# liuli33/CMLPL

Measured on AMD Instinct MI355X. Metric: HSI patches/sec per training step, higher is better.
Workload: dtype f32 (convolutions: f32 operands as 3 exact bf16 pieces on the bf16 MFMA, 6 of 9 piece products, f32 accumulate, per-product worst case 2^-21 -- conv1's tap loops of the per-sample kernels as 2 fp16 pieces with power-of-two operand scales, 3 piece products, worst case 2^-20 / mean 2^-23, falling back; 1 GPU; B2: synthetic PaviaU-shaped patches 11x11x103, spectrum 103, 9 classes, 128 labelled + 128 unlabelled rows per GPU (batch 256), dual BaseNet2 fwd/bwd + contrastive/mutual losses + bank + Adam, epoch 1 (memory-bank smoothing active), in-kernel PCG4D noise / Philox dropout; global_batch=256, parallelism=dp1

## Files before the change

### cmlpl_amd/csrc/conv0.hip

```cpp
#include "common.hpp"
#include "kernels.hpp"
#include "gemm_tn.hpp"

namespace cmlpl {

constexpr int C0_KMAX = 128;

template <int KCAP>
__global__ __launch_bounds__(256) void conv0_fwd_kernel(const float* __restrict__ xn, const float* __restrict__ w0t,
                                                        long long w0t_ns, const float* __restrict__ b,
                                                        long long pstride, float* __restrict__ a0, int n, int C,
                                                        int HW) {
  extern __shared__ __attribute__((aligned(16))) float wl[];
  const int tid = threadIdx.x, lane = tid & 63, l31 = lane & 31, hh = lane >> 5;
  const int wave = __builtin_amdgcn_readfirstlane(tid >> 6);
  const int net = blockIdx.y;
  const int Cp = (C + 1) & ~1, KK = Cp >> 1;
  const long long M = (long long)n * HW;
  const long long m = ((long long)blockIdx.x * 4 + wave) * 32 + l31;
  const long long mm = (m < M) ? m : 0;
  const int sample = (int)(mm / HW), pix = (int)(mm - (long long)sample * HW);
  const float* ap = xn + ((long long)net * n + sample) * C * HW + pix;
  float av[KCAP];
#pragma unroll
  for (int q = 0; q < KCAP; ++q) {
    const int c = 2 * q + hh;
    const bool ok = (q < KK) && (c < C);
    const float v = ap[(long long)(ok ? c : 0) * HW];
    av[q] = ok ? v : 0.f;
  }
  const float4* wsrc = (const float4*)(w0t + (long long)net * w0t_ns);
  staged_copy<8, float4>(Cp * 16, tid, [&](int i) { return wsrc[i]; }, [&](int i, float4 v) { ((float4*)wl)[i] = v; });
  __syncthreads();
  f32x16 acc0 = zero16(), acc1 = zero16();
#pragma unroll
  for (int q = 0; q < KCAP; ++q) {
    if (q < KK) {
      const int c = 2 * q + hh;
      acc0 = mfma32(av[q], wl[c * 64 + l31], acc0);
      acc1 = mfma32(av[q], wl[c * 64 + 32 + l31], acc1);
    }
  }
  const float* bias = b + (long long)net * pstride;
  const float bv0 = bias[l31], bv1 = bias[32 + l31];
  const long long mbase = ((long long)blockIdx.x * 4 + wave) * 32;
  float* out = a0 + (long long)net * M * 64;
#pragma unroll
  for (int r = 0; r < 16; ++r) {
    const long long mr = mbase + acc_row(r, lane);
    if (mr < M) {
      out[mr * 64 + l31] = acc0[r] + bv0;
      out[mr * 64 + 32 + l31] = acc1[r] + bv1;
    }
  }
}

hipError_t launch_conv0_fwd(int nets, int n, int C, int HW, const float* xn, const float* w0t, long long w0t_ns,
                            const float* b, long long pstride, float* a0, hipStream_t st) {
  const long long M = (long long)n * HW;
  const int KK = ((C + 1) & ~1) / 2;
  if (KK > C0_KMAX) return hipErrorInvalidValue;
  const size_t lds = (size_t)2 * KK * 64 * 4;
  dim3 grid((unsigned)((M + 127) / 128), nets);
  if (KK <= 32)      hipLaunchKernelGGL((conv0_fwd_kernel<32>), grid, dim3(256), lds, st, xn, w0t, w0t_ns, b, pstride, a0, n, C, HW);
  else if (KK <= 64) hipLaunchKernelGGL((conv0_fwd_kernel<64>), grid, dim3(256), lds, st, xn, w0t, w0t_ns, b, pstride, a0, n, C, HW);
  else               hipLaunchKernelGGL((conv0_fwd_kernel<128>), grid, dim3(256), lds, st, xn, w0t, w0t_ns, b, pstride, a0, n, C, HW);
  return hipGetLastError();
}

constexpr int C0A_SP = 132;
struct Conv0aArgs {
  XSrc xs; const float* w0b3; long long w0b3_ns; const float* b; long long pstride;
  float* a0; float* xn;
  int n, C, HW;
};

template <int KQMAX>
__global__ __launch_bounds__(256, KQMAX <= 4 ? 4 : 2) void conv0a_fwd_kernel(Conv0aArgs a) {
  extern __shared__ __attribute__((aligned(16))) float slab[];
  const int tid = threadIdx.x, lane = tid & 63, l31 = lane & 31, hh = lane >> 5;
  const int wave = __builtin_amdgcn_readfirstlane(tid >> 6);
  const int s = blockIdx.y, net = blockIdx.z, p0 = blockIdx.x * 128;
  const int C = a.C, HW = a.HW, KQ0 = (C + 15) >> 4;
  const int npx = (HW - p0 < 128) ? HW - p0 : 128, np8 = npx >> 3;
  const long long per = (long long)C * HW;
  const float* xrow = xsrc_row(a.xs, net, s, per);
  const float sigma = a.xs.sigma;
  const float* nzrow = (sigma != 0.f) ? xsrc_noise_row(a.xs, net, s, per) : nullptr;
  const uint64_t gs = xsrc_global_sample(a.xs, s), rstep = xsrc_step(a.xs);
  float* xnrow = (a.xn != nullptr) ? a.xn + ((long long)net * a.n + s) * per : nullptr;
  const uint4* wq = (const uint4*)(a.w0b3 + (long long)net * a.w0b3_ns) + lane;
  constexpr int NI = (KQMAX * 16 * 16 + 255) / 256;
  const int items = C * np8;
  const uint32_t mg = (np8 <= 1) ? 0u : (uint32_t)((0x100000000ULL + (uint32_t)np8 - 1) / (uint32_t)np8);
  float4 v0[NI], v1[NI];
  int cc[NI], jj[NI];
#pragma unroll
  for (int q = 0; q < NI; ++q) {
    const int it = tid + 256 * q;
    const int itc = it < items ? it : 0;
    cc[q] = mg == 0u ? itc : (int)__umulhi((uint32_t)itc, mg);
    jj[q] = itc - cc[q] * np8;
    const float* src = xrow + (long long)cc[q] * HW + p0 + 8 * jj[q];
    v0[q] = *(const float4*)src; v1[q] = *(const float4*)(src + 4);
  }
  if (sigma != 0.f) {
#pragma unroll
    for (int q = 0; q < NI; ++q) {
      const long long e = (long long)cc[q] * HW + p0 + 8 * jj[q];
      float4 z0, z1;
      if (nzrow != nullptr) { z0 = *(const float4*)(nzrow + e); z1 = *(const float4*)(nzrow + e + 4); }
      else noise_normal8(a.xs.seed, rstep, STREAM_NOISE_XP + net, gs, (uint32_t)(e >> 3), z0, z1);
      v0[q].x = fmaf(z0.x, sigma, v0[q].x); v0[q].y = fmaf(z0.y, sigma, v0[q].y);
      v0[q].z = fmaf(z0.z, sigma, v0[q].z); v0[q].w = fmaf(z0.w, sigma, v0[q].w);
      v1[q].x = fmaf(z1.x, sigma, v1[q].x); v1[q].y = fmaf(z1.y, sigma, v1[q].y);
      v1[q].z = fmaf(z1.z, sigma, v1[q].z); v1[q].w = fmaf(z1.w, sigma, v1[q].w);
    }
  }
#pragma unroll
  for (int q = 0; q < NI; ++q) {
    if (tid + 256 * q < items) {
      float* d = slab + cc[q] * C0A_SP + 8 * jj[q];
      *(float4*)d = v0[q]; *(float4*)(d + 4) = v1[q];
      if (xnrow != nullptr) {
        float* g = xnrow + (long long)cc[q] * HW + p0 + 8 * jj[q];
        *(float4*)g = v0[q]; *(float4*)(g + 4) = v1[q];
      }
    }
  }
  uint4 bw[2][6];
#pragma unroll
  for (int kq = 0; kq < 2; ++kq)
#pragma unroll
    for (int i = 0; i < 6; ++i) bw[kq][i] = wq[(((kq < KQ0 ? kq : 0) * 3 + (i >> 1)) * 2 + (i & 1)) * 64];
  for (int i = C * C0A_SP + tid; i < KQ0 * 16 * C0A_SP; i += 256) slab[i] = 0.f;
  if (npx < 128)
    for (int i = tid; i < C * (128 - npx); i += 256) { const int c = i / (128 - npx); slab[c * C0A_SP + npx + (i - c * (128 - npx))] = 0.f; }
  __syncthreads();
  if (32 * wave >= npx) return;
  f32x16 z0 = zero16(), z1 = zero16();
  const float* ap = slab + 8 * hh * C0A_SP + 32 * wave + l31;
  float rn[8];
#pragma unroll
  for (int j = 0; j < 8; ++j) rn[j] = ap[j * C0A_SP];
#pragma unroll
  for (int kq = 0; kq < KQMAX; ++kq) {
    if (kq < KQ0) {
      uint4 A1, A2, A3;
      a_split(make_float4(rn[0], rn[1], rn[2], rn[3]), make_float4(rn[4], rn[5], rn[6], rn[7]), A1, A2, A3);
      if (kq + 1 < KQ0) {
#pragma unroll
        for (int j = 0; j < 8; ++j) rn[j] = ap[((kq + 1) * 16 + j) * C0A_SP];
      }
      const uint4 (&b)[6] = bw[kq & 1];
      z0 = mfma_b3(A1, A2, A3, b[0], b[2], b[4], z0);
      z1 = mfma_b3(A1, A2, A3, b[1], b[3], b[5], z1);
      if (kq + 2 < KQ0) {
#pragma unroll
        for (int i = 0; i < 6; ++i) bw[kq & 1][i] = wq[(((kq + 2) * 3 + (i >> 1)) * 2 + (i & 1)) * 64];
      }
    }
  }
  const float* bias = a.b + (long long)net * a.pstride;
  const float bv0 = bias[l31], bv1 = bias[32 + l31];
  float* out = a.a0 + (((long long)net * a.n + s) * HW + p0 + 32 * wave) * 64;
#pragma unroll
  for (int r = 0; r < 16; ++r) {
    const int m = acc_row(r, lane);
    if (32 * wave + m < npx) {
      out[(long long)m * 64 + l31] = z0[r] + bv0;
      out[(long long)m * 64 + 32 + l31] = z1[r] + bv1;
    }
  }
}

bool conv0a_ok(int C, int HW) {
  return switches().conv0a != 0 && C >= 1 && C <= 128 && (HW & 7) == 0 && HW >= 8;
}

hipError_t launch_conv0a_fwd(int nets, int n, int C, int HW, const XSrc& xs, const float* w0b3, long long w0b3_ns,
                             const float* b, long long pstride, float* a0, float* xn, hipStream_t st) {
  if (!conv0a_ok(C, HW)) return hipErrorInvalidValue;
  Conv0aArgs a;
  a.xs = xs; a.w0b3 = w0b3; a.w0b3_ns = w0b3_ns; a.b = b; a.pstride = pstride; a.a0 = a0; a.xn = xn;
  a.n = n; a.C = C; a.HW = HW;
  const int KQ0 = (C + 15) / 16;
  const size_t lds = (size_t)KQ0 * 16 * C0A_SP * 4;
  static DevOnce attr_once;
  hipError_t e = ensure_max_lds(attr_once, conv0a_fwd_kernel<4>, conv0a_fwd_kernel<8>);
  if (e != hipSuccess) return e;
  dim3 grid((HW + 127) / 128, n, nets);
  if (KQ0 <= 4) hipLaunchKernelGGL((conv0a_fwd_kernel<4>), grid, dim3(256), lds, st, a);
  else          hipLaunchKernelGGL((conv0a_fwd_kernel<8>), grid, dim3(256), lds, st, a);
  return hipGetLastError();
}

constexpr int C0_MAXT = 4;
constexpr int C0_PB = 8;

typedef __attribute__((address_space(3))) void c0_lds_void;
typedef __attribute__((address_space(1))) const void c0_gbl_void;
template <bool DMA>
__global__ __launch_bounds__(256) void conv0_wgrad_kernel(const float* __restrict__ xn, const float* __restrict__ da0,
                                                          float* __restrict__ part, int n, int C, int HWfull, int G,
                                                          int PS, const uint32_t* __restrict__ zstat,
                                                          const uint32_t* __restrict__ h2flag, long long h2flag_ns) {
  extern __shared__ __attribute__((aligned(16))) float smem[];
  const int tid = threadIdx.x, lane = tid & 63, l31 = lane & 31, hh = lane >> 5;
  const int wave = __builtin_amdgcn_readfirstlane(tid >> 6);
  const int net = blockIdx.y, g = blockIdx.x;
  const int NT = (C + 31) >> 5, Ct = NT * 32;
  const int HW = HWfull / PS;
  const int HWp = DMA ? HW : ((HW + 2) | 1);
  const int SPG = (n + G - 1) / G;
  const int sbeg = g * SPG, send = (sbeg + SPG < n) ? sbeg + SPG : n;
  const int ct = wave & 1, it0 = wave >> 1;
  f32x16 acc[C0_MAXT];
#pragma unroll
  for (int t = 0; t < C0_MAXT; ++t) acc[t] = zero16();
  float dbacc = 0.f;
  for (int i = (DMA ? C * HW : 0) + tid; i < Ct * HWp + 64; i += 256) smem[i] = 0.f;
  const int pairs = (HW + 1) >> 1;

  const bool zflag = zstat != nullptr && h2flag[(long long)net * h2flag_ns] == 0u;
  for (int su = sbeg * PS; su < send * PS; ++su) {
    const int s = su / PS, p0 = (su - s * PS) * HW;
    if (zflag && zstat[(2 * 2 + net) * n + s] == 0u && (zstat[(0 * 2 + net) * n + s] >> 23) < 255u) continue;
    const float* brow = da0 + (((long long)net * n + s) * HWfull + p0) * 64 + ct * 32 + l31;
    float bq[4][C0_PB];
    auto fetch = [&](float (&buf)[C0_PB], int t0) {
#pragma unroll
      for (int q = 0; q < C0_PB; ++q) {
        const int p = 2 * (t0 + q) + hh;
        buf[q] = brow[(long long)(p < HW ? p : 0) * 64];
      }
    };
    fetch(bq[0], 0); fetch(bq[1], C0_PB); fetch(bq[2], 2 * C0_PB);
    __syncthreads();
    const float* xs = xn + ((long long)net * n + s) * C * HWfull + p0;
    if (DMA) {
      const int nf4 = (C * HW) >> 2;
      for (int q = wave; q * 64 < nf4; q += 4) {
        const int f = q * 64 + lane;
        if (f < nf4)
          __builtin_amdgcn_global_load_lds((c0_gbl_void*)(xs + 4 * f), (c0_lds_void*)(smem + q * 256), 16, 0, 0);
      }
      const int rem = C * HW - 4 * nf4;
      if (tid < rem) smem[4 * nf4 + tid] = xs[4 * nf4 + tid];
    } else {
      if ((HW & 3) == 0) {
        const int H4 = HW >> 2;
        staged_copy<8, float4>(C * H4, tid,
                               [&](int i) { const int c = i / H4, q = i - c * H4; return *(const float4*)(xs + (long long)c * HWfull + 4 * q); },
                               [&](int i, float4 v) {
                                 const int c = i / H4, p = 4 * (i - c * H4);
                                 float* d = smem + c * HWp + p;
                                 d[0] = v.x; d[1] = v.y; d[2] = v.z; d[3] = v.w;
                               });
      } else {
        staged_copy<16, float>(C * HW, tid, [&](int i) { const int c = i / HW; return xs[(long long)c * HWfull + (i - c * HW)]; },
                               [&](int i, float v) { const int c = i / HW, p = i - c * HW; smem[c * HWp + p] = v; });
      }
    }
    __syncthreads();
    for (int t1 = 0; t1 < pairs; t1 += 4 * C0_PB) {
#pragma unroll
      for (int u = 0; u < 4; ++u) {
        const int t0 = t1 + u * C0_PB;
        if (t0 + 3 * C0_PB < pairs) fetch(bq[(u + 3) & 3], t0 + 3 * C0_PB);
        if (t0 < pairs) {
          float bv[C0_PB];
#pragma unroll
          for (int q = 0; q < C0_PB; ++q) {
            const int p = 2 * (t0 + q) + hh;
            bv[q] = (t0 + q < pairs && p < HW) ? bq[u][q] : 0.f;
            dbacc += bv[q];
          }
#pragma unroll
          for (int k = 0; k < C0_MAXT; ++k) {
            const int tile = it0 + 2 * k;
            if (tile < NT) {
              const float* xr = smem + (tile * 32 + l31) * HWp + 2 * t0 + hh;
              float av[C0_PB];
#pragma unroll
              for (int q = 0; q < C0_PB; ++q) av[q] = xr[2 * q];
              __builtin_amdgcn_sched_barrier(0);
#pragma unroll
              for (int q = 0; q < C0_PB; ++q) acc[k] = mfma32(av[q], bv[q], acc[k]);
            }
          }
        }
      }
    }
  }
  const int Cw = conv0_partial_rows(C);
  float* pp = part + ((long long)net * G + g) * ((long long)Cw * 64 + 64);
#pragma unroll
  for (int k = 0; k < C0_MAXT; ++k) {
    const int tile = it0 + 2 * k;
    if (tile < NT) {
#pragma unroll
      for (int r = 0; r < 16; ++r) {
        const int row = tile * 32 + acc_row(r, lane);
        if (row < Cw) pp[row * 64 + ct * 32 + l31] = acc[k][r];
      }
    }
  }
  if (it0 == 0) {
    const float tot = dbacc + __shfl_xor(dbacc, 32, 64);
    if (hh == 0) pp[(long long)Cw * 64 + ct * 32 + l31] = tot;
  }
}

__device__ __forceinline__ float4 part_row(const float* p, int g, int G, int PS) {
  uint32_t keep = g < G ? 0xffffffffu : 0u;
  asm volatile("" : "+v"(keep));
  const float4 x = *(const float4*)(p + (size_t)(g < G ? g : 0) * PS);
  return make_float4(__uint_as_float(__float_as_uint(x.x) & keep), __uint_as_float(__float_as_uint(x.y) & keep),
                     __uint_as_float(__float_as_uint(x.z) & keep), __uint_as_float(__float_as_uint(x.w) & keep));
}
__device__ __forceinline__ void add_quad(float4& s, const float4& a, const float4& b, const float4& c, const float4& d) {
  s.x += (a.x + b.x) + (c.x + d.x); s.y += (a.y + b.y) + (c.y + d.y);
  s.z += (a.z + b.z) + (c.z + d.z); s.w += (a.w + b.w) + (c.w + d.w);
}

__device__ __forceinline__ float conv0_fold(const ReduceProb& pr, int eb, int net, float4* red4) {
  const int tid = threadIdx.x, col = tid & 31, h = (tid >> 5) & 1, sl = tid >> 6;
  const int G = pr.G, PS = pr.PS;
  const int e0 = eb + col * 4;
  const float* p = pr.part + (long long)net * G * PS + (e0 < PS ? e0 : 0);
  float4 s = make_float4(0.f, 0.f, 0.f, 0.f);
  for (int g0 = sl + 16 * h; g0 - 16 * h < G; g0 += 128) {
    const float4 a0 = part_row(p, g0, G, PS), a1 = part_row(p, g0 + 4, G, PS);
    const float4 a2 = part_row(p, g0 + 8, G, PS), a3 = part_row(p, g0 + 12, G, PS);
    const float4 b0 = part_row(p, g0 + 32, G, PS), b1 = part_row(p, g0 + 36, G, PS);
    const float4 b2 = part_row(p, g0 + 40, G, PS), b3 = part_row(p, g0 + 44, G, PS);
    const float4 c0 = part_row(p, g0 + 64, G, PS), c1 = part_row(p, g0 + 68, G, PS);
    const float4 c2 = part_row(p, g0 + 72, G, PS), c3 = part_row(p, g0 + 76, G, PS);
    const float4 d0 = part_row(p, g0 + 96, G, PS), d1 = part_row(p, g0 + 100, G, PS);
    const float4 d2 = part_row(p, g0 + 104, G, PS), d3 = part_row(p, g0 + 108, G, PS);
    add_quad(s, a0, a1, a2, a3);
    add_quad(s, b0, b1, b2, b3);
    add_quad(s, c0, c1, c2, c3);
    add_quad(s, d0, d1, d2, d3);
  }
  red4[tid] = s;
  __syncthreads();
  const float* sm = (const float*)red4;
  const int w = tid & 127;
  return ((sm[w] + sm[128 + w]) + (sm[256 + w] + sm[384 + w])) + ((sm[512 + w] + sm[640 + w]) + (sm[768 + w] + sm[896 + w]));
}

__device__ __forceinline__ void partial_reduce_block(const ReduceTable& t, int bx, int net, float (*red)[64]) {
  int pi = 0;
  if (t.count > 1 && bx >= t.p[1].blk0) pi = 1;
  if (t.count > 2 && bx >= t.p[2].blk0) pi = 2;
  const ReduceProb pr = t.p[pi];
  const int tid = threadIdx.x, el = tid & 63, sl = tid >> 6;
  if (t.dyn_cursor != nullptr && bx == 0 && net == 0 && tid == 0) {
    const int c = *t.dyn_cursor + 1;
    *t.dyn_cursor = c;
    const uint4* src = (const uint4*)(t.dyn_table + c);
    uint4* dst = (uint4*)t.dyn_table;
    const uint4 r0 = src[0], r1 = src[1], r2 = src[2], r3 = src[3];
    dst[0] = r0; dst[1] = r1; dst[2] = r2; dst[3] = r3;
  }
  const int G = pr.G, PS = pr.PS;
  const int body = PS - 64;
  if (pr.mode == 0) {
    const int eb = (bx - pr.blk0) * REDUCE_CONV0_EL, e = eb + tid;
    const float sum = conv0_fold(pr, eb, net, (float4*)&red[0][0]);
    if (tid < REDUCE_CONV0_EL && e < PS) {
      if (e >= body) pr.db[(long long)net * t.grad_ns + (e - body)] = sum;
      else if ((e >> 6) < pr.C) pr.dW[(long long)net * t.grad_ns + (e & 63) * pr.C + (e >> 6)] = sum;
    }
    return;
  }
  const int e0 = ((bx - pr.blk0) * 64 + el) * 4;
  const bool ev = e0 < PS;
  const float* p = pr.part + (long long)net * G * PS + (ev ? e0 : 0);
  float4 s0 = make_float4(0.f, 0.f, 0.f, 0.f), s1 = s0;
  for (int g0 = sl; g0 < G; g0 += 64) {
    const float4 a0 = part_row(p, g0, G, PS), a1 = part_row(p, g0 + 4, G, PS);
    const float4 a2 = part_row(p, g0 + 8, G, PS), a3 = part_row(p, g0 + 12, G, PS);
    const float4 a4 = part_row(p, g0 + 16, G, PS), a5 = part_row(p, g0 + 20, G, PS);
    const float4 a6 = part_row(p, g0 + 24, G, PS), a7 = part_row(p, g0 + 28, G, PS);
    const float4 b0 = part_row(p, g0 + 32, G, PS), b1 = part_row(p, g0 + 36, G, PS);
    const float4 b2 = part_row(p, g0 + 40, G, PS), b3 = part_row(p, g0 + 44, G, PS);
    const float4 b4 = part_row(p, g0 + 48, G, PS), b5 = part_row(p, g0 + 52, G, PS);
    const float4 b6 = part_row(p, g0 + 56, G, PS), b7 = part_row(p, g0 + 60, G, PS);
    add_quad(s0, a0, a1, a2, a3); add_quad(s1, a4, a5, a6, a7);
    add_quad(s0, b0, b1, b2, b3); add_quad(s1, b4, b5, b6, b7);
  }
  float4* red4 = (float4*)&red[0][0];
  red4[sl * 64 + el] = make_float4(s0.x + s1.x, s0.y + s1.y, s0.z + s1.z, s0.w + s1.w);
  __syncthreads();
  if (sl == 0 && ev) {
    const float4 a = red4[el], b = red4[64 + el], c = red4[128 + el], d = red4[192 + el];
    const float sum[4] = {(a.x + b.x) + (c.x + d.x), (a.y + b.y) + (c.y + d.y), (a.z + b.z) + (c.z + d.z),
                          (a.w + b.w) + (c.w + d.w)};
#pragma unroll
    for (int j = 0; j < 4; ++j) {
      const int e = e0 + j;
      if (e >= body) {
        pr.db[(long long)net * t.grad_ns + (e - body)] = sum[j];
      } else {
        const int s = e >> 12, ci = (e >> 6) & 63, co = e & 63;
        pr.dW[(long long)net * t.grad_ns + co * 576 + ci * 9 + s] = sum[j];
      }
    }
  }
}

__global__ __launch_bounds__(256) void partial_reduce_kernel(ReduceTable t) {
  __shared__ __attribute__((aligned(16))) float red[16][64];
  partial_reduce_block(t, (int)blockIdx.x, (int)blockIdx.y, red);
}

__global__ __launch_bounds__(256) void reduce_gemm_kernel(ReduceTable t, int reduce_blocks, GemmTN2 g) {
  __shared__ GemmTNShared sh;
  const int bid = (int)blockIdx.x;
  if (bid < reduce_blocks) partial_reduce_block(t, bid % t.total_blocks, bid / t.total_blocks, (float (*)[64])&sh.red[0][0][0]);
  else gemm_tn_block(g, bid - reduce_blocks, sh);
}

__device__ __forceinline__ int red_swz(int col) { return col ^ (((col >> 4) & 7) << 1); }

__device__ __forceinline__ void reduce_adam_block_conv0(const ReduceTable& t, const ReduceProb& pr, int bx, int net,
                                                        float* sm, const AdamFuse& f) {
  const int tid = threadIdx.x;
  const int PS = pr.PS, body = PS - 64;
  const int eb = (bx - pr.blk0) * REDUCE_CONV0_EL, e = eb + tid, c = e >> 6, co = e & 63;
  long long po = -1;
  if (tid < REDUCE_CONV0_EL && e < PS) {
    if (e >= body) po = (pr.db - f.gbase) + (e - body);
    else if (c < pr.C) po = (pr.dW - f.gbase) + (long long)co * pr.C + c;
  }
  float* const pp = f.params + (long long)net * f.pstride;
  float* const pm = f.m + (long long)net * f.pstride;
  float* const pv = f.v + (long long)net * f.pstride;
  const long long o = po < 0 ? 0 : po;
  float mq = pm[o], vq = pv[o];
  const float pq = pp[o];
  const float sum = conv0_fold(pr, eb, net, (float4*)sm);
  if (po < 0) return;
  const_cast<float*>(f.gbase)[(long long)net * t.grad_ns + po] = sum;
  const float pn = adam_update<true, false>(mq, vq, pq, sum, f, 1.f, f.keep);
  pm[po] = mq; pv[po] = vq; pp[po] = pn;
  if (e < body) {
    float* const pkn = f.packed + (long long)net * f.pi.stride;
    pkn[pack_off_w0t() + c * 64 + co] = pn;
    uint32_t pcs[3];
    b3_split(pn, pcs);
    uint16_t* wb = (uint16_t*)(pkn + pack_off_w0b3(f.pi.C, f.pi.bands));
#pragma unroll
    for (int pc = 0; pc < 3; ++pc) wb[conv_b3_index(0, c, co, pc)] = (uint16_t)pcs[pc];
  }
}

__device__ __forceinline__ void reduce_adam_block(const ReduceTable& t, int bx, int net, float* sm, const AdamFuse& f) {
  int pi = 0;
  if (t.count > 1 && bx >= t.p[1].blk0) pi = 1;
  if (t.count > 2 && bx >= t.p[2].blk0) pi = 2;
  const ReduceProb pr = t.p[pi];
  if (pr.mode == 0) { reduce_adam_block_conv0(t, pr, bx, net, sm, f); return; }
  const int tid = threadIdx.x, lane = tid & 63, el = lane, sl = tid >> 6;
  const int G = pr.G, PS = pr.PS, body = PS - 64;
  const int eb = (bx - pr.blk0) * REDUCE_FUSED_EL;
  const bool conv3 = eb < body;
  const long long offW = pr.dW - f.gbase, offB = pr.db - f.gbase;
  int u[2];
  long long po[2];
#pragma unroll
  for (int q = 0; q < 2; ++q) {
    if (conv3) {
      const int cil = lane & 7, co = (sl * 2 + q) * 8 + (lane >> 3);
      u[q] = cil * 64 + co;
      const int e = eb + u[q];
      po[q] = offW + co * 576 + ((e >> 6) & 63) * 9 + (e >> 12);
    } else {
      u[q] = tid + 256 * q;
      const int e = eb + u[q];
      if (e >= PS) po[q] = -1;
      else if (e >= body) po[q] = offB + (e - body);
      else po[q] = offW + (e & 63) * 576 + ((e >> 6) & 63) * 9 + (e >> 12);
    }
  }
  float* const pp = f.params + (long long)net * f.pstride;
  float* const pm = f.m + (long long)net * f.pstride;
  float* const pv = f.v + (long long)net * f.pstride;
  float mq[2], vq[2], pq[2];
#pragma unroll
  for (int q = 0; q < 2; ++q) {
    const long long o = po[q] < 0 ? 0 : po[q];
    mq[q] = pm[o]; vq[q] = pv[o]; pq[q] = pp[o];
  }
  const float* p[2];
#pragma unroll
  for (int c = 0; c < 2; ++c) {
    const int e0 = eb + (el + 64 * c) * 4;
    p[c] = pr.part + (long long)net * G * PS + (e0 < PS ? e0 : 0);
  }
  float4 s0[2], s1[2];
  s0[0] = s0[1] = s1[0] = s1[1] = make_float4(0.f, 0.f, 0.f, 0.f);
  for (int g0 = sl; g0 < G; g0 += 32) {
    float4 v[2][8];
#pragma unroll
    for (int c = 0; c < 2; ++c) {
#pragma unroll
      for (int q = 0; q < 8; ++q) {
        v[c][q] = part_row(p[c], g0 + 4 * q, G, PS);
      }
    }
#pragma unroll
    for (int c = 0; c < 2; ++c) {
#define CMLPL_ADD4(F) s0[c].F += (v[c][0].F + v[c][1].F) + (v[c][2].F + v[c][3].F); s1[c].F += (v[c][4].F + v[c][5].F) + (v[c][6].F + v[c][7].F);
      CMLPL_ADD4(x) CMLPL_ADD4(y) CMLPL_ADD4(z) CMLPL_ADD4(w)
#undef CMLPL_ADD4
    }
  }
  float4* red4 = (float4*)sm;
#pragma unroll
  for (int c = 0; c < 2; ++c)
    red4[sl * 128 + red_swz(el + 64 * c)] = make_float4(s0[c].x + s1[c].x, s0[c].y + s1[c].y, s0[c].z + s1[c].z, s0[c].w + s1[c].w);
  __syncthreads();
  float* const wl = sm + 2048;
  float* const gr = const_cast<float*>(f.gbase) + (long long)net * t.grad_ns;
  float* const pkn = f.packed + (long long)net * f.pi.stride;
#pragma unroll
  for (int q = 0; q < 2; ++q) {
    if (po[q] < 0) continue;
    const int w = 4 * red_swz(u[q] >> 2) + (u[q] & 3);
    const float sum = (sm[w] + sm[512 + w]) + (sm[1024 + w] + sm[1536 + w]);
    gr[po[q]] = sum;
    const float pn = conv3 ? adam_update<true, true>(mq[q], vq[q], pq[q], sum, f, 1.f, f.keep)
                           : adam_update<true, false>(mq[q], vq[q], pq[q], sum, f, 1.f, f.keep);
    pm[po[q]] = mq[q]; pv[po[q]] = vq[q]; pp[po[q]] = pn;
    if (conv3) wl[(u[q] & 63) * 9 + (u[q] >> 6)] = pn;
  }
  if (!conv3) return;
  __syncthreads();
  const int which = (offW == f.pi.off_w2) ? 2 : 0, tap = eb >> 12, ci0 = (eb >> 6) & 63;
  static_assert(H2_WEXP == 13, "h2_split_w scales by 2^13");
  bool bad = false;
  if (tid < 64) {
    const int co = tid;
    uint4* bf = (uint4*)(pkn + pack_off_b3(f.pi.C, f.pi.bands, which));
    uint4* hf = (uint4*)(pkn + pack_off_h2(f.pi.C, f.pi.bands, which));
    uint32_t pc[8][3], ph[8][2];
#pragma unroll
    for (int j = 0; j < 8; ++j) {
      const float w = wl[co * 9 + j];
      b3_split(w, pc[j]);
      bad |= h2_split_w(w, ph[j]);
    }
#pragma unroll
    for (int pcs = 0; pcs < 3; ++pcs)
      bf[conv_b3_index(tap, ci0, co, pcs) >> 3] =
          make_uint4(pc[0][pcs] | (pc[1][pcs] << 16), pc[2][pcs] | (pc[3][pcs] << 16),
                     pc[4][pcs] | (pc[5][pcs] << 16), pc[6][pcs] | (pc[7][pcs] << 16));
#pragma unroll
    for (int pcs = 0; pcs < 2; ++pcs)
      hf[conv_h2_index(tap, ci0, co, pcs) >> 3] =
          make_uint4(ph[0][pcs] | (ph[1][pcs] << 16), ph[2][pcs] | (ph[3][pcs] << 16),
                     ph[4][pcs] | (ph[5][pcs] << 16), ph[6][pcs] | (ph[7][pcs] << 16));
  } else if (tid < 64 + 128) {
    const int it = tid - 64, co0 = (it & 15) * 4, cil = it >> 4, ci = ci0 + cil;
    uint2* bd = (uint2*)(pkn + pack_off_b3(f.pi.C, f.pi.bands, which + 1));
    uint2* hd = (uint2*)(pkn + pack_off_h2(f.pi.C, f.pi.bands, which + 1));
    uint32_t pc[4][3], ph[4][2];
#pragma unroll
    for (int j = 0; j < 4; ++j) {
      const float w = wl[(co0 + j) * 9 + cil];
      b3_split(w, pc[j]);
      bad |= h2_split_w(w, ph[j]);
    }
#pragma unroll
    for (int pcs = 0; pcs < 3; ++pcs)
      bd[conv_b3_index(8 - tap, co0, ci, pcs) >> 2] = make_uint2(pc[0][pcs] | (pc[1][pcs] << 16), pc[2][pcs] | (pc[3][pcs] << 16));
#pragma unroll
    for (int pcs = 0; pcs < 2; ++pcs)
      hd[conv_h2_index(8 - tap, co0, ci, pcs) >> 2] = make_uint2(ph[0][pcs] | (ph[1][pcs] << 16), ph[2][pcs] | (ph[3][pcs] << 16));
  }
  if (bad) atomicOr((unsigned int*)(pkn + pack_off_h2flag(f.pi.C, f.pi.bands)), 1u);
}

__global__ __launch_bounds__(256) void reduce_gemm_adam_kernel(ReduceTable t, int reduce_blocks, GemmTN2 g, AdamFuse f) {
  __shared__ GemmTNShared sh;
  __shared__ float x0[16][64];
  const int bid = (int)blockIdx.x;
  if (bid < reduce_blocks) reduce_adam_block(t, bid % t.total_blocks, bid / t.total_blocks, &sh.red[0][0][0], f);
  else gemm_tn_block<true>(g, bid - reduce_blocks, sh, &f, x0);
}

hipError_t launch_reduce_gemm(int nets, const ReduceTable& t, const GemmTN& g0, const GemmTN& g1, hipStream_t st,
                              const AdamFuse* fu) {
  GemmTN2 g;
  g.p[0] = g0; g.p[1] = g1; g.nblk0 = gemm_tn_blocks(g0);
  const int rb = t.total_blocks * nets, gb = g.nblk0 + gemm_tn_blocks(g1);
  for (int i = 0; i < t.count; ++i)
    if (t.p[i].el != reduce_el(t.p[i].mode, fu != nullptr)) return hipErrorInvalidValue;
  if (fu != nullptr) {
    if (t.dyn_cursor != nullptr) return hipErrorInvalidValue;
    hipLaunchKernelGGL(reduce_gemm_adam_kernel, dim3(rb + gb), dim3(256), 0, st, t, rb, g, *fu);
  } else {
    hipLaunchKernelGGL(reduce_gemm_kernel, dim3(rb + gb), dim3(256), 0, st, t, rb, g);
  }
  return hipGetLastError();
}

void reduce_table_add(ReduceTable& t, const float* part, int G, int PS, int mode, int C, float* dW, float* db, bool fused) {
  const int el = reduce_el(mode, fused);
  ReduceProb& p = t.p[t.count++];
  p.part = part; p.dW = dW; p.db = db; p.G = G; p.PS = PS; p.mode = mode; p.C = C; p.blk0 = t.total_blocks;
  p.el = el;
  t.total_blocks += (PS + el - 1) / el;
}

hipError_t launch_partial_reduce(int nets, const ReduceTable& t, hipStream_t st) {
  for (int i = 0; i < t.count; ++i)
    if (t.p[i].el != reduce_el(t.p[i].mode, false)) return hipErrorInvalidValue;
  hipLaunchKernelGGL(partial_reduce_kernel, dim3(t.total_blocks, nets), dim3(256), 0, st, t);
  return hipGetLastError();
}

int conv0_partial_size(int C) { return conv0_partial_rows(C) * 64 + 64; }

int plan_conv0_wgrad_G(int n, int C, int HW) {
  (void)C; (void)HW;
  int G = n < 256 ? n : 256;
  return G < 1 ? 1 : G;
}

hipError_t launch_conv0_wgrad(int nets, int n, int C, int HW, const float* xn, const float* da0, float* part,
                              hipStream_t st, const uint32_t* zstat, const uint32_t* h2flag, long long h2flag_ns) {
  if (switches().zero_skip == 0 || h2flag == nullptr) zstat = nullptr;
  const int NT = (C + 31) / 32, Ct = NT * 32;
  if (NT > 2 * C0_MAXT) return hipErrorInvalidValue;
  const bool dma_off = switches().conv0_dma == 0;
  const bool dma = (HW & 1) && !dma_off;
  const int force_ps = switches().conv0_ps;
  int PS = (!dma && (HW & 7) == 0 && ((size_t)Ct * ((HW + 2) | 1) + 64) * 4 > LDS_MAX / 2) ? 2 : 1;
  if (force_ps == 1 || (force_ps == 2 && !dma && (HW & 7) == 0)) PS = force_ps;
  const int HWs = HW / PS;
  const int HWp = dma ? HW : ((HWs + 2) | 1);
  const size_t lds = ((size_t)Ct * HWp + 64) * 4;
  if (lds > LDS_MAX) return hipErrorInvalidValue;
  static DevOnce attr_once;
  {
    hipError_t e = ensure_max_lds(attr_once, conv0_wgrad_kernel<false>, conv0_wgrad_kernel<true>);
    if (e != hipSuccess) return e;
  }
  const int G = plan_conv0_wgrad_G(n, C, HW);
  if (dma) hipLaunchKernelGGL(conv0_wgrad_kernel<true>, dim3(G, nets), dim3(256), lds, st, xn, da0, part, n, C, HW, G, 1, zstat, h2flag, h2flag_ns);
  else     hipLaunchKernelGGL(conv0_wgrad_kernel<false>, dim3(G, nets), dim3(256), lds, st, xn, da0, part, n, C, HW, G, PS, zstat, h2flag, h2flag_ns);
  return hipGetLastError();
}

}
```

### cmlpl_amd/csrc/gemm_tn.hpp

```cpp
#pragma once
#include "common.hpp"
#include "kernels.hpp"

namespace cmlpl {

constexpr int GT_DEPTH = 16;

struct GemmTN2 { GemmTN p[2]; int nblk0; };
struct GemmTNShared { __attribute__((aligned(16))) float red[3][16][64]; float ared[4][64]; };

__device__ __forceinline__ float mul_alone(float a, float b) {
  float r = a * b;
  asm volatile("" : "+v"(r));
  return r;
}

template <bool OPT, bool CHUNK, class A>
__device__ __forceinline__ float adam_update(float& mm, float& vv, float p, float g, const A& a, float coef, float keep) {
  if (OPT) {
    g = mul_alone(g, coef);
    p = mul_alone(p, keep);
    mm = fmaf(a.w1, g - mm, mm);
    vv = CHUNK ? fmaf(g, a.w2 * g, vv * a.b2) : fmaf(vv, a.b2, (a.w2 * g) * g);
    const float denom = sqrtf(vv) / a.bc2_sqrt + a.eps;
    return fmaf(-a.step_size, mm / denom, p);
  }

  mm = mm + a.w1 * (g - mm);
  vv = vv * a.b2 + (a.w2 * g) * g;
  const float denom = sqrtf(vv) / a.bc2_sqrt + a.eps;
  return p - a.step_size * (mm / denom);
}

template <bool UPD = false>
__device__ __forceinline__ void gemm_tn_block(const GemmTN2& t, int bid, GemmTNShared& sh, const AdamFuse* f = nullptr,
                                              float (*x0)[64] = nullptr) {
  const int tid = threadIdx.x, lane = tid & 63, l31 = lane & 31, hh = lane >> 5;
  const int wave = __builtin_amdgcn_readfirstlane(tid >> 6);
  const int pi = (bid >= t.nblk0) ? 1 : 0;
  const GemmTN g = t.p[pi];
  int b = bid - (pi ? t.nblk0 : 0);
  const int NTg = (g.N + 31) >> 5, MTg = (g.M + 31) >> 5;
  const int nt = b % NTg; b /= NTg;
  const int mt = b % MTg;
  const int bz = b / MTg;
  const float* A = g.A + (long long)bz * g.a_bstride;
  const float* B = g.B + (long long)bz * g.b_bstride;
  const int i = mt * 32 + l31, j = nt * 32 + l31;
  const bool iv = i < g.M, jv = j < g.N;
  const float* ap = A + (iv ? i : 0);
  const float* bp = B + (jv ? j : 0);
  const int R = g.R;
  const int pairs = (R + 1) >> 1;
  const int ppw = (pairs + 3) >> 2;
  const int t0 = wave * ppw, t1 = (t0 + ppw < pairs) ? t0 + ppw : pairs;
  f32x16 acc = zero16();
  float asum = 0.f;
  float um[4], uv[4], up[4], bm = 0.f, bv2 = 0.f, bpar = 0.f, bg = 0.f;
  long long uoff = 0, boff = 0;
  bool bias_upd = false;
  if (UPD) {
    uoff = (long long)bz * f->pstride + (g.C - f->gbase);
#pragma unroll
    for (int rr = 0; rr < 4; ++rr) {
      const int row = mt * 32 + acc_row(4 * wave + rr, lane);
      const long long o = uoff + ((jv && row < g.M) ? (long long)row * g.ldc + j : 0);
      um[rr] = f->m[o]; uv[rr] = f->v[o]; up[rr] = f->params[o];
    }
    bias_upd = wave == 0 && g.bias != nullptr && nt == 0 && hh == 0 && i < ((g.M + 3) & ~3);
    if (bias_upd) {
      boff = (long long)bz * f->pstride + (g.bias - f->gbase) + i;
      bm = f->m[boff]; bv2 = f->v[boff]; bpar = f->params[boff];
      if (!iv) bg = g.bias[(long long)bz * g.bias_bstride + i];
    }
  }
  for (int tb = t0; tb < t1; tb += GT_DEPTH) {
    float av[GT_DEPTH], bv[GT_DEPTH];
    int seg = 0, off = 0;
    if (g.b_seg_rows > 0) { const int r0 = 2 * tb + hh; seg = r0 / g.b_seg_rows; off = r0 - seg * g.b_seg_rows; }
#pragma unroll
    for (int q = 0; q < GT_DEPTH; ++q) {
      const int r = 2 * (tb + q) + hh;
      const bool rv = (tb + q < t1) && (r < R);
      const int rc = rv ? r : 0;
      const long long bo = g.b_seg_rows > 0 ? (rv ? (long long)seg * g.b_seg_stride + (long long)off * g.ldb : 0)
                                            : (long long)rc * g.ldb;
      const float a = ap[(long long)rc * g.lda], b = bp[bo];
      av[q] = (rv && iv) ? a : 0.f;
      bv[q] = (rv && jv) ? b : 0.f;
      off += 2;
      while (g.b_seg_rows > 0 && off >= g.b_seg_rows) { off -= g.b_seg_rows; ++seg; }
    }
#pragma unroll
    for (int q = 0; q < GT_DEPTH; ++q) {
      asum += av[q];
      acc = mfma32(av[q], bv[q], acc);
    }
  }
  if (wave > 0) {
#pragma unroll
    for (int r = 0; r < 16; ++r) sh.red[wave - 1][r][lane] = acc[r];
  }
  if (UPD && wave == 0) {
#pragma unroll
    for (int r = 0; r < 16; ++r) x0[r][lane] = acc[r];
  }
  sh.ared[wave][lane] = asum;
  __syncthreads();
  if (UPD) {
    float* C = g.C + (long long)bz * g.c_bstride;
    if (jv) {
#pragma unroll
      for (int rr = 0; rr < 4; ++rr) {
        const int r = 4 * wave + rr, row = mt * 32 + acc_row(r, lane);
        float v = (((x0[r][lane] + sh.red[0][r][lane]) + sh.red[1][r][lane]) + sh.red[2][r][lane]) * g.scale;
        if (g.bias_in != nullptr) v += g.bias_in[(long long)bz * g.bias_in_bstride + j];
        if (g.relu) v = relu_nan(v);
        if (row < g.M) {
          const long long o = uoff + (long long)row * g.ldc + j;
          C[(long long)row * g.ldc + j] = v;
          const float pn = adam_update<true, false>(um[rr], uv[rr], up[rr], v, *f, 1.f, f->keep);
          f->m[o] = um[rr]; f->v[o] = uv[rr]; f->params[o] = pn;
        }
      }
    }
    if (wave == 0 && g.bias != nullptr && nt == 0) {
      float tot = (sh.ared[0][lane] + sh.ared[1][lane]) + (sh.ared[2][lane] + sh.ared[3][lane]);
      tot += __shfl_xor(tot, 32, 64);
      if (hh == 0 && iv) g.bias[(long long)bz * g.bias_bstride + i] = tot * g.scale;
      if (bias_upd) {
        const float pn = adam_update<true, false>(bm, bv2, bpar, iv ? tot * g.scale : bg, *f, 1.f, f->keep);
        f->m[boff] = bm; f->v[boff] = bv2; f->params[boff] = pn;
      }
    }
    return;
  }
  if (wave == 0) {
    float* C = g.C + (long long)bz * g.c_bstride;
    if (jv) {
#pragma unroll
      for (int r = 0; r < 16; ++r) {
        const int row = mt * 32 + acc_row(r, lane);
        float v = (((acc[r] + sh.red[0][r][lane]) + sh.red[1][r][lane]) + sh.red[2][r][lane]) * g.scale;
        if (g.bias_in != nullptr) v += g.bias_in[(long long)bz * g.bias_in_bstride + j];
        if (g.relu) v = relu_nan(v);
        if (row < g.M) C[(long long)row * g.ldc + j] = v;
      }
    }
    if (g.bias != nullptr && nt == 0) {
      float tot = (sh.ared[0][lane] + sh.ared[1][lane]) + (sh.ared[2][lane] + sh.ared[3][lane]);
      tot += __shfl_xor(tot, 32, 64);
      if (hh == 0 && iv) g.bias[(long long)bz * g.bias_bstride + i] = tot * g.scale;
    }
  }
}

inline int gemm_tn_blocks(const GemmTN& g) { return ((g.M + 31) / 32) * ((g.N + 31) / 32) * g.batches; }

}
```

Baseline: 1.807 million patches/s.

## Double-buffer TN GEMM row loads and put GEMM blocks first in fused grid

Rewrites the TN GEMM inner loop as a two-stage software pipeline. Two register buffers of loads are kept in flight while MFMAs consume the previous batch, and pointer offsets are stepped incrementally instead of recomputed per row. The Adam state and bias_in loads are moved into a tail issued alongside the first loads, so their latency overlaps the GEMM. The fused reduce+GEMM kernels now assign the low block indices to GEMM blocks so those longer blocks dispatch first. This costs extra registers, which may reduce occupancy.

```diff
diff --git a/cmlpl_amd/csrc/conv0.hip b/cmlpl_amd/csrc/conv0.hip
--- a/cmlpl_amd/csrc/conv0.hip
+++ b/cmlpl_amd/csrc/conv0.hip
@@ -419,9 +419,9 @@
 
 __global__ __launch_bounds__(256) void reduce_gemm_kernel(ReduceTable t, int reduce_blocks, GemmTN2 g) {
   __shared__ GemmTNShared sh;
-  const int bid = (int)blockIdx.x;
-  if (bid < reduce_blocks) partial_reduce_block(t, bid % t.total_blocks, bid / t.total_blocks, (float (*)[64])&sh.red[0][0][0]);
-  else gemm_tn_block(g, bid - reduce_blocks, sh);
+  const int gemm_blocks = (int)gridDim.x - reduce_blocks, bid = (int)blockIdx.x - gemm_blocks;
+  if (bid >= 0) partial_reduce_block(t, bid % t.total_blocks, bid / t.total_blocks, (float (*)[64])&sh.red[0][0][0]);
+  else gemm_tn_block(g, (int)blockIdx.x, sh);
 }
 
 __device__ __forceinline__ int red_swz(int col) { return col ^ (((col >> 4) & 7) << 1); }
@@ -588,9 +588,9 @@
 __global__ __launch_bounds__(256) void reduce_gemm_adam_kernel(ReduceTable t, int reduce_blocks, GemmTN2 g, AdamFuse f) {
   __shared__ GemmTNShared sh;
   __shared__ float x0[16][64];
-  const int bid = (int)blockIdx.x;
-  if (bid < reduce_blocks) reduce_adam_block(t, bid % t.total_blocks, bid / t.total_blocks, &sh.red[0][0][0], f);
-  else gemm_tn_block<true>(g, bid - reduce_blocks, sh, &f, x0);
+  const int gemm_blocks = (int)gridDim.x - reduce_blocks, bid = (int)blockIdx.x - gemm_blocks;
+  if (bid >= 0) reduce_adam_block(t, bid % t.total_blocks, bid / t.total_blocks, &sh.red[0][0][0], f);
+  else gemm_tn_block<true>(g, (int)blockIdx.x, sh, &f, x0);
 }
 
 hipError_t launch_reduce_gemm(int nets, const ReduceTable& t, const GemmTN& g0, const GemmTN& g1, hipStream_t st,
diff --git a/cmlpl_amd/csrc/gemm_tn.hpp b/cmlpl_amd/csrc/gemm_tn.hpp
--- a/cmlpl_amd/csrc/gemm_tn.hpp
+++ b/cmlpl_amd/csrc/gemm_tn.hpp
@@ -30,6 +30,86 @@
   vv = vv * a.b2 + (a.w2 * g) * g;
   const float denom = sqrtf(vv) / a.bc2_sqrt + a.eps;
   return p - a.step_size * (mm / denom);
+}
+
+template <bool SEG>
+struct GemmTNWalk {
+  const float* ap; const float* bp;
+  long long oa, ob, sa, sb;
+  int kn, klim;
+  int seg, off, seg_rows, ldb; long long seg_stride;
+  bool iv, jv;
+
+  __device__ __forceinline__ GemmTNWalk(const GemmTN& g, const float* ap_, const float* bp_, bool iv_, bool jv_, int hh,
+                                        int t0, int t1)
+      : ap(ap_), bp(bp_), oa((long long)(2 * t0 + hh) * g.lda), ob((long long)(2 * t0 + hh) * g.ldb), sa(2LL * g.lda),
+        sb(2LL * g.ldb), kn(t0), seg(0), off(0), seg_rows(g.b_seg_rows), ldb(g.ldb), seg_stride(g.b_seg_stride),
+        iv(iv_), jv(jv_) {
+    const int rows = (g.R - hh + 1) >> 1;
+    klim = t1 < rows ? t1 : rows;
+    if (SEG) { const int r0 = 2 * t0 + hh; seg = r0 / seg_rows; off = r0 - seg * seg_rows; }
+  }
+  __device__ __forceinline__ void request(float (&a)[GT_DEPTH], float (&b)[GT_DEPTH]) {
+#pragma unroll
+    for (int q = 0; q < GT_DEPTH; ++q) {
+      const bool rv = kn + q < klim;
+      if (SEG) {
+        ob = (long long)seg * seg_stride + (long long)off * ldb;
+        off += 2;
+        while (off >= seg_rows) { off -= seg_rows; ++seg; }
+      }
+      a[q] = ap[rv ? oa : 0];
+      b[q] = bp[rv ? ob : 0];
+      oa += sa;
+      if (!SEG) ob += sb;
+      asm volatile("" : "+v"(oa), "+v"(ob));
+      __builtin_amdgcn_sched_barrier(0);
+    }
+    kn += GT_DEPTH;
+  }
+  __device__ __forceinline__ void run(const float (&a)[GT_DEPTH], const float (&b)[GT_DEPTH], int kb, f32x16& acc,
+                                      float& asum) const {
+#pragma unroll
+    for (int q = 0; q < GT_DEPTH; ++q) {
+      const bool rv = kb + q < klim;
+      const float x = (rv && iv) ? a[q] : 0.f, y = (rv && jv) ? b[q] : 0.f;
+      asum += x;
+      acc = mfma32(x, y, acc);
+    }
+  }
+};
+
+template <bool SEG, class Tail>
+__device__ __forceinline__ void gemm_tn_rows(const GemmTN& g, const float* ap, const float* bp, bool iv, bool jv, int hh,
+                                             int t0, int t1, f32x16& acc, float& asum, Tail&& tail) {
+  GemmTNWalk<SEG> w(g, ap, bp, iv, jv, hh, t0, t1);
+  float a0[GT_DEPTH], b0[GT_DEPTH], a1[GT_DEPTH], b1[GT_DEPTH];
+  if (t0 + GT_DEPTH >= t1) {
+    if (t0 < t1) w.request(a0, b0);
+    tail();
+    __builtin_amdgcn_sched_barrier(0);
+    if (t0 < t1) w.run(a0, b0, t0, acc, asum);
+    return;
+  }
+  w.request(a0, b0);
+  w.request(a1, b1);
+  tail();
+  __builtin_amdgcn_sched_barrier(0);
+  int tb = t0;
+  while (tb + 2 * GT_DEPTH < t1) {
+    asm volatile("" : "+v"(w.klim));
+    w.run(a0, b0, tb, acc, asum);
+    __builtin_amdgcn_sched_barrier(0);
+    w.request(a0, b0);
+    __builtin_amdgcn_sched_barrier(0);
+    w.run(a1, b1, tb + GT_DEPTH, acc, asum);
+    __builtin_amdgcn_sched_barrier(0);
+    w.request(a1, b1);
+    __builtin_amdgcn_sched_barrier(0);
+    tb += 2 * GT_DEPTH;
+  }
+  w.run(a0, b0, tb, acc, asum);
+  if (tb + GT_DEPTH < t1) w.run(a1, b1, tb + GT_DEPTH, acc, asum);
 }
 
 template <bool UPD = false>
@@ -56,47 +136,29 @@
   const int t0 = wave * ppw, t1 = (t0 + ppw < pairs) ? t0 + ppw : pairs;
   f32x16 acc = zero16();
   float asum = 0.f;
-  float um[4], uv[4], up[4], bm = 0.f, bv2 = 0.f, bpar = 0.f, bg = 0.f;
+  float um[4], uv[4], up[4], bm = 0.f, bv2 = 0.f, bpar = 0.f, bg = 0.f, bin = 0.f;
   long long uoff = 0, boff = 0;
   bool bias_upd = false;
-  if (UPD) {
-    uoff = (long long)bz * f->pstride + (g.C - f->gbase);
-#pragma unroll
-    for (int rr = 0; rr < 4; ++rr) {
-      const int row = mt * 32 + acc_row(4 * wave + rr, lane);
-      const long long o = uoff + ((jv && row < g.M) ? (long long)row * g.ldc + j : 0);
-      um[rr] = f->m[o]; uv[rr] = f->v[o]; up[rr] = f->params[o];
-    }
-    bias_upd = wave == 0 && g.bias != nullptr && nt == 0 && hh == 0 && i < ((g.M + 3) & ~3);
-    if (bias_upd) {
-      boff = (long long)bz * f->pstride + (g.bias - f->gbase) + i;
-      bm = f->m[boff]; bv2 = f->v[boff]; bpar = f->params[boff];
-      if (!iv) bg = g.bias[(long long)bz * g.bias_bstride + i];
-    }
-  }
-  for (int tb = t0; tb < t1; tb += GT_DEPTH) {
-    float av[GT_DEPTH], bv[GT_DEPTH];
-    int seg = 0, off = 0;
-    if (g.b_seg_rows > 0) { const int r0 = 2 * tb + hh; seg = r0 / g.b_seg_rows; off = r0 - seg * g.b_seg_rows; }
-#pragma unroll
-    for (int q = 0; q < GT_DEPTH; ++q) {
-      const int r = 2 * (tb + q) + hh;
-      const bool rv = (tb + q < t1) && (r < R);
-      const int rc = rv ? r : 0;
-      const long long bo = g.b_seg_rows > 0 ? (rv ? (long long)seg * g.b_seg_stride + (long long)off * g.ldb : 0)
-                                            : (long long)rc * g.ldb;
-      const float a = ap[(long long)rc * g.lda], b = bp[bo];
-      av[q] = (rv && iv) ? a : 0.f;
-      bv[q] = (rv && jv) ? b : 0.f;
-      off += 2;
-      while (g.b_seg_rows > 0 && off >= g.b_seg_rows) { off -= g.b_seg_rows; ++seg; }
-    }
-#pragma unroll
-    for (int q = 0; q < GT_DEPTH; ++q) {
-      asum += av[q];
-      acc = mfma32(av[q], bv[q], acc);
-    }
-  }
+  auto tail = [&]() {
+    if (g.bias_in != nullptr && (UPD || wave == 0)) bin = g.bias_in[(long long)bz * g.bias_in_bstride + (jv ? j : 0)];
+    if (UPD) {
+      uoff = (long long)bz * f->pstride + (g.C - f->gbase);
+#pragma unroll
+      for (int rr = 0; rr < 4; ++rr) {
+        const int row = mt * 32 + acc_row(4 * wave + rr, lane);
+        const long long o = uoff + ((jv && row < g.M) ? (long long)row * g.ldc + j : 0);
+        um[rr] = f->m[o]; uv[rr] = f->v[o]; up[rr] = f->params[o];
+      }
+      bias_upd = wave == 0 && g.bias != nullptr && nt == 0 && hh == 0 && i < ((g.M + 3) & ~3);
+      if (bias_upd) {
+        boff = (long long)bz * f->pstride + (g.bias - f->gbase) + i;
+        bm = f->m[boff]; bv2 = f->v[boff]; bpar = f->params[boff];
+        if (!iv) bg = g.bias[(long long)bz * g.bias_bstride + i];
+      }
+    }
+  };
+  if (g.b_seg_rows > 0) gemm_tn_rows<true>(g, ap, bp, iv, jv, hh, t0, t1, acc, asum, tail);
+  else gemm_tn_rows<false>(g, ap, bp, iv, jv, hh, t0, t1, acc, asum, tail);
   if (wave > 0) {
 #pragma unroll
     for (int r = 0; r < 16; ++r) sh.red[wave - 1][r][lane] = acc[r];
@@ -114,7 +176,7 @@
       for (int rr = 0; rr < 4; ++rr) {
         const int r = 4 * wave + rr, row = mt * 32 + acc_row(r, lane);
         float v = (((x0[r][lane] + sh.red[0][r][lane]) + sh.red[1][r][lane]) + sh.red[2][r][lane]) * g.scale;
-        if (g.bias_in != nullptr) v += g.bias_in[(long long)bz * g.bias_in_bstride + j];
+        if (g.bias_in != nullptr) v += bin;
         if (g.relu) v = relu_nan(v);
         if (row < g.M) {
           const long long o = uoff + (long long)row * g.ldc + j;
@@ -142,7 +204,7 @@
       for (int r = 0; r < 16; ++r) {
         const int row = mt * 32 + acc_row(r, lane);
         float v = (((acc[r] + sh.red[0][r][lane]) + sh.red[1][r][lane]) + sh.red[2][r][lane]) * g.scale;
-        if (g.bias_in != nullptr) v += g.bias_in[(long long)bz * g.bias_in_bstride + j];
+        if (g.bias_in != nullptr) v += bin;
         if (g.relu) v = relu_nan(v);
         if (row < g.M) C[(long long)row * g.ldc + j] = v;
       }
```

Measured after the change: 1.839 million patches/s, median of 6. +1.8%, better.
